# MachinaIO/mxx

Hardware: AMD Instinct MI355X
Metric: dcrt_ring_ops_per_s (higher is better)
Workload: dtype u32

## Files before the change

### mxx_amd/csrc/common.h

```cpp
#pragma once

#include <hip/hip_runtime.h>

#include <atomic>
#include <cstddef>
#include <cstdint>
#include <cstdio>
#include <exception>
#include <map>
#include <unordered_map>
#include <mutex>
#include <string>
#include <vector>

#include "../../include/gpupoly.h"

constexpr size_t GPUPOLY_MAX_LIMBS = 64;

struct LimbConst {
    uint64_t q;
    uint64_t mu;
    uint64_t mu64;
    uint64_t n_inv;
    uint64_t n_inv_sh;
    uint64_t mu32;
    uint64_t inv_last_w;
    uint64_t inv_last_w_sh;
    uint32_t kbits;
    uint32_t lazy_terms;
};

struct EnvSwitches {
    int ntt_path = 0;
    int ntt14 = 0;
    bool decompose_fused = true;
    char matmul_path = 0;
    int matmul_tile = 0;
    bool gsamp_simple = false;
    bool gsamp_no_uni = false;
    bool p1_simple = false;
    int sampler_per_lane = 0;
    int sampler_fill_every = 0;
    bool ntt64_int = false;
    int ntt_phase = 0;
    bool serde_general = false;
    bool rng_compat = false;
    bool pack24 = true;
    int skinny24 = 0;
    int skinny24_shape = 0;
    size_t mul_decompose_many_budget = 0;
    size_t mul_decompose_pairs_budget = 0;
    size_t gadget_scalar_budget = 0;
    size_t ggh15_lookup_budget = 0;
    char mul_sum_path = 0;
    size_t crt_recompose_chunk_bytes = size_t(256) << 20;
    void load();
};

struct GpuContext {
    EnvSwitches env;
    int device = 0;
    std::vector<int> gpu_ids;
    uint32_t logN = 0;
    int N = 0;
    int level = 0;
    uint32_t dnum = 0;
    int limb_count = 0;
    bool wide = false;
    int word_bytes = 4;
    uint32_t crt_bits = 0;
    std::vector<uint64_t> moduli;
    hipStream_t stream = nullptr;
    LimbConst *d_limbs = nullptr;
    LimbConst *d_limbs_r = nullptr;
    void *d_tw_fwd = nullptr;
    void *d_tw_fwd_sh = nullptr;
    void *d_tw_inv = nullptr;
    void *d_tw_inv_sh = nullptr;
    void *d_tw2_fwd = nullptr;
    void *d_tw2_inv = nullptr;
    bool lazy_ok = false;
    bool tight_ok = false;
    void *d_tw2s_inv = nullptr;
    bool signed_ok = false;
    void *d_twf_fwd = nullptr, *d_twf_inv = nullptr;
    void *d_flimbs = nullptr;
    bool f64_ok = false;
    uint64_t *d_garner = nullptr;
    std::vector<uint64_t> garner_inv;
    std::vector<LimbConst> limbs;
    hipEvent_t timer_start = nullptr, timer_stop = nullptr;
    std::vector<hipEvent_t> marks;
    std::mutex mutex;
    bool pool_ok = false;
    std::mutex alloc_mutex;
    std::multimap<size_t, void *> free_blocks;
    std::unordered_map<void *, size_t> live_blocks;
    size_t cached_bytes = 0, cache_limit = 0;
    std::atomic<const char *> last_kernel{""};
    bool pack24_ok = false;
    std::mutex layout_mutex;
    std::map<uint32_t, void *> gadget_weights;
    std::map<std::vector<uint64_t>, void *> gadget_const_tables;
};

struct LayoutTag {
    std::atomic<int> v{GPU_MATRIX_LAYOUT_WORDS};
    LayoutTag() = default;
    LayoutTag(const LayoutTag &o) : v(o.v.load(std::memory_order_acquire)) {}
    LayoutTag &operator=(const LayoutTag &o) {
        v.store(o.v.load(std::memory_order_acquire), std::memory_order_release);
        return *this;
    }
};

struct GpuMatrix {
    GpuContext *ctx = nullptr;
    int level = 0;
    size_t rows = 0, cols = 0;
    int format = GPU_POLY_FORMAT_EVAL;
    void *storage = nullptr;
    size_t bytes = 0;
    LayoutTag layout;
    bool borrowed = false;
    GpuMatrix *parent = nullptr;
    int views = 0;
};

struct GpuEventSet {
    std::vector<hipEvent_t> events;
    int device = 0;
    void *staging = nullptr;
    GpuContext *ctx = nullptr;
    void *dev_staging = nullptr;
};

struct GpuP1CovarianceCache {
    GpuContext *ctx = nullptr;
    int level = 0;
    size_t d = 0, m = 0, n = 0;
    double sigma = 0, s = 0, dgg_stddev = 0;
    double *sqrt_var = nullptr;
    double *update_coeff = nullptr;
    void *karney_div = nullptr;
};

struct P1KeyEntry {
    const double *sqrt_var;
    const double *update_coeff;
    const void *karney_div;
};

static inline dim3 item_grid(size_t items, unsigned threads) {
    const size_t blocks = (items + threads - 1) / threads;
    const size_t max_x = (static_cast<size_t>(1) << 31) / threads;
    if (blocks <= max_x) return dim3(static_cast<unsigned>(blocks ? blocks : 1));
    const size_t y = (blocks + max_x - 1) / max_x;
    return dim3(static_cast<unsigned>((blocks + y - 1) / y), static_cast<unsigned>(y));
}
#if defined(__HIPCC__)
__device__ __forceinline__ size_t item_index() {
    return (static_cast<size_t>(blockIdx.y) * gridDim.x + blockIdx.x) * blockDim.x + threadIdx.x;
}
#endif

extern std::atomic<uint64_t> g_kernel_launches;
extern std::atomic<int> g_trace_on;
void trace_launch_begin(const char *name, hipStream_t stream, dim3 grid, dim3 block);
void trace_launch_end(hipStream_t stream);
void trace_set_bytes(double bytes);
#define MXX_TRACE_BYTES(b)                                                                        \
    do {                                                                                          \
        if (g_trace_on.load(std::memory_order_relaxed)) trace_set_bytes(static_cast<double>(b)); \
    } while (0)
#define MXX_LAUNCH(kern, grid, block, lds, strm, ...)                          \
    do {                                                                       \
        g_kernel_launches.fetch_add(1, std::memory_order_relaxed);             \
        const bool mxx_tr_ = g_trace_on.load(std::memory_order_relaxed) != 0;  \
        if (mxx_tr_) trace_launch_begin(#kern, strm, grid, block);             \
        hipLaunchKernelGGL(kern, grid, block, lds, strm, __VA_ARGS__);         \
        if (mxx_tr_) trace_launch_end(strm);                                   \
    } while (0)
#define MXX_TRACED_COPY(name, strm, bytes, stmt)                               \
    do {                                                                       \
        const bool mxx_tr_ = g_trace_on.load(std::memory_order_relaxed) != 0;  \
        if (mxx_tr_) {                                                         \
            trace_set_bytes(static_cast<double>(bytes));                       \
            trace_launch_begin(name, strm, dim3(0), dim3(0));                  \
        }                                                                      \
        stmt;                                                                  \
        if (mxx_tr_) trace_launch_end(strm);                                   \
    } while (0)

int set_error(const char *msg);
int set_error(const std::string &msg);
int set_error(hipError_t err, const char *what);

#define HIP_TRY(expr)                                          \
    do {                                                       \
        hipError_t _e = (expr);                                \
        if (_e != hipSuccess) return set_error(_e, #expr);     \
    } while (0)

template <auto... KERNELS>
static int lds_opt_in(const GpuContext *ctx, size_t lds) {
    static std::atomic<uint64_t> configured{0};
    const uint64_t bit = 1ull << (ctx->device & 63);
    if (lds <= 64 * 1024 || (configured.load() & bit)) return 0;
    for (const void *f : {reinterpret_cast<const void *>(KERNELS)...})
        HIP_TRY(hipFuncSetAttribute(f, hipFuncAttributeMaxDynamicSharedMemorySize, static_cast<int>(lds)));
    configured.fetch_or(bit);
    return 0;
}

extern int (*g_roctx_push)(const char *);
extern int (*g_roctx_pop)();
void roctx_init_once();
struct RoctxScope {
    bool on;
    explicit RoctxScope(const char *name) {
        roctx_init_once();
        on = g_roctx_push != nullptr;
        if (on) g_roctx_push(name);
    }
    ~RoctxScope() {
        if (on) g_roctx_pop();
    }
};

#define ABI_GUARD_BEGIN try { RoctxScope roctx_scope_(__func__);
#define ABI_GUARD_END                                                         \
    }                                                                         \
    catch (const std::exception &e) { return set_error(e.what()); }           \
    catch (...) { return set_error("unknown exception in libgpupoly"); }

inline size_t matrix_polys(const GpuMatrix *m) { return m->rows * m->cols; }
inline size_t matrix_limbs(const GpuMatrix *m) { return static_cast<size_t>(m->level) + 1; }
inline size_t matrix_words(const GpuMatrix *m) { return matrix_polys(m) * matrix_limbs(m) * static_cast<size_t>(m->ctx->N); }

void *words_ptr(const GpuMatrix *m);
const void *packed24_ptr(const GpuMatrix *m, bool *packed);
inline size_t packed24_bytes(const GpuMatrix *m) { return m->bytes / 4 * 3; }
inline bool storage_overlaps(const GpuMatrix *x, const GpuMatrix *y) {
    if (x == y) return true;
    if (!x->storage || !y->storage || x->bytes == 0 || y->bytes == 0) return false;
    const size_t xb = x->layout.v.load(std::memory_order_acquire) == GPU_MATRIX_LAYOUT_PACKED24 ? packed24_bytes(x) : x->bytes;
    const size_t yb = y->layout.v.load(std::memory_order_acquire) == GPU_MATRIX_LAYOUT_PACKED24 ? packed24_bytes(y) : y->bytes;
    const char *xs = static_cast<const char *>(x->storage), *ys = static_cast<const char *>(y->storage);
    return xs < ys + yb && ys < xs + xb;
}
inline bool same_block(const GpuMatrix *x, const GpuMatrix *y) {
    return x == y || (x->storage == y->storage && x->bytes == y->bytes);
}
inline bool partial_overlap(const GpuMatrix *out, const GpuMatrix *operand) {
    return storage_overlaps(out, operand) && !same_block(out, operand);
}
inline bool row_block_overlaps(const GpuMatrix *m, size_t row, size_t rows, const GpuMatrix *y) {
    if (m->layout.v.load(std::memory_order_acquire) == GPU_MATRIX_LAYOUT_PACKED24) return rows && m->cols && storage_overlaps(m, y);
    if (!m->storage) return false;
    const size_t poly_bytes = matrix_limbs(m) * static_cast<size_t>(m->ctx->N) * m->ctx->word_bytes;
    GpuMatrix block;
    block.storage = static_cast<char *>(m->storage) + row * m->cols * poly_bytes;
    block.bytes = rows * m->cols * poly_bytes;
    return storage_overlaps(&block, y);
}
bool pack24_eligible(const GpuMatrix *m);
int pack24_store(GpuMatrix *m, bool ntt);

int sample_impl(GpuMatrix *out, int dist, double sigma, GpuRngSeed seed, size_t full_ncol, size_t col_offset, bool keep_coeff,
                size_t row_offset = 0, uint32_t tower_first = 0, uint32_t tower_count = 0);

struct RngBlockWindow {
    size_t cols, full_ncol, col_offset;
};
int sample_blocks_impl(const char *entry, bool hashed, GpuMatrix *out, int dist_type, const GpuRngSeed *seeds, const GpuHashTags *tags,
                       size_t nblk, int layout, const size_t *seg_cols, const RngBlockWindow *win, const double *sigma = nullptr);
int sample_decomposed_blocks_impl(const char *entry, bool hashed, GpuMatrix *out, int dist_type, const GpuRngSeed *seeds,
                                  const GpuHashTags *tags, size_t nblk, uint32_t base_bits, int small, size_t src_rows, size_t full_ncol,
                                  size_t col_offset);

int hash_tags_check(const char *entry, const GpuHashTags *tags, size_t ntags, size_t *table_bytes);
size_t hash_tags_staged_words(const GpuHashTags *tags, size_t ntags, size_t table_bytes);
void hash_tags_stage(const GpuHashTags *tags, size_t ntags, size_t table_bytes, uint64_t *staging);
int launch_hash_seeds(GpuContext *ctx, GpuRngSeed *d_seeds, const GpuHashTags *tags, size_t ntags, const uint64_t *d_staged);

int ctx_activate(const GpuContext *ctx);
bool ctx_is_registered(const GpuContext *ctx);
int ctx_alloc(GpuContext *ctx, size_t bytes, void **out);
void ctx_free(GpuContext *ctx, void *ptr);
struct CtxBlock {
    GpuContext *ctx;
    void *ptr = nullptr;
    explicit CtxBlock(GpuContext *c) : ctx(c) {}
    CtxBlock(const CtxBlock &) = delete;
    CtxBlock &operator=(const CtxBlock &) = delete;
    ~CtxBlock() {
        if (ptr) ctx_free(ctx, ptr);
    }
    int alloc(size_t bytes) { return ctx_alloc(ctx, bytes, &ptr); }
    void *release() {
        void *p = ptr;
        ptr = nullptr;
        return p;
    }
};
int matrix_check_same_shape(const GpuMatrix *a, const GpuMatrix *b, const char *who);
int coeff_domain_source(const GpuMatrix *mat, CtxBlock &scratch, const void **src);

int launch_ntt(GpuContext *ctx, void *data, size_t vectors, int limbs_per_poly, bool inverse);
int launch_ntt_lds_u32(GpuContext *ctx, uint32_t *data, size_t vectors, uint32_t L, bool inverse);
int launch_ntt_digits_u32(GpuContext *ctx, uint32_t *out, const uint32_t *coeff, size_t out_vectors, uint32_t L,
                          uint32_t src_cols, uint32_t towers, uint32_t dpt, uint32_t base_bits, size_t k, uint32_t td0 = 0);
int launch_ntt_lds_u64(GpuContext *ctx, uint64_t *data, size_t vectors, uint32_t L, bool inverse);
int launch_ntt_digits_u64(GpuContext *ctx, uint64_t *out, const uint64_t *coeff, size_t out_vectors, uint32_t L,
                          uint32_t src_cols, uint32_t towers, uint32_t dpt, uint32_t base_bits, size_t k, uint32_t td0 = 0);
int launch_intt_oop_u32(GpuContext *ctx, uint32_t *out, const uint32_t *in, size_t vectors, uint32_t L);
int launch_ntt_add_u32(GpuContext *ctx, uint32_t *out, const uint32_t *src, const uint32_t *add, size_t vectors, uint32_t L);
int launch_mul_intt_u32(GpuContext *ctx, uint32_t *out, const uint32_t *in, const uint32_t *w, size_t vectors, uint32_t L);
int launch_matmul(GpuMatrix *out, const GpuMatrix *lhs, const GpuMatrix *rhs);
int launch_ntt_fwd_pack24_u32(GpuContext *ctx, uint32_t *out, const uint32_t *in, size_t vectors, uint32_t L);
int launch_matmul_skinny24(GpuMatrix *out, const GpuMatrix *lhs, const GpuMatrix *rhs, bool small_grid);
int skinny24_parse_shape(const char *s);
int launch_matmul_dma_u32(GpuMatrix *out, const GpuMatrix *lhs, const GpuMatrix *rhs);
int launch_matmul_dma32_u32(GpuMatrix *out, const GpuMatrix *lhs, const GpuMatrix *rhs);
int launch_matmul_mfma_u32(GpuMatrix *out, const GpuMatrix *lhs, const GpuMatrix *rhs);
int launch_copy_block(GpuMatrix *out, const GpuMatrix *src, size_t dst_row, size_t dst_col, size_t src_row,
                      size_t src_col, size_t rows, size_t cols, bool add);
int sample_p1_keyed_segments(const GpuP1CovarianceCache *cache, const P1KeyEntry *d_keys, const GpuMatrix *tp2,
                             const GpuRngSeed *seeds, const size_t *seg_cols, size_t nseg, GpuMatrix *out);
int launch_scatter_i64(GpuMatrix *out, const int64_t *vals);
int finish_staged_i64(GpuMatrix *out, CtxBlock &stage, hipError_t launch_err, const char *what, bool transform = true);
```

### mxx_amd/csrc/matmul_skinny24.hip

```cpp
#include "common.h"
#include "matmul_tile.h"
#include "modarith.h"

#include <map>
#include <string>

namespace skinny24 {

typedef uint32_t u32x3 __attribute__((ext_vector_type(3)));
typedef uint32_t u32x4 __attribute__((ext_vector_type(4)));

__device__ __forceinline__ __amdgpu_buffer_rsrc_t row_rsrc(const char *base, uint32_t bytes) {
    return __builtin_amdgcn_make_buffer_rsrc(const_cast<char *>(base), 0, static_cast<int>(bytes), 0x00020000);
}
constexpr int kAuxNT = 2;

__device__ __forceinline__ void unpack4(uint32_t w0, uint32_t w1, uint32_t w2, uint32_t *o) {
    o[0] = w0 & 0xffffffu;
    o[1] = __builtin_amdgcn_alignbit(w1, w0, 24) & 0xffffffu;
    o[2] = __builtin_amdgcn_alignbit(w2, w1, 16) & 0xffffffu;
    o[3] = w2 >> 8;
}

template <int TC, int G, int WPE, int MAP>
__global__ void __launch_bounds__(256, WPE)
    kernel(uint32_t *__restrict__ C, const uint32_t *__restrict__ A, const uint32_t *__restrict__ B, const LimbConst *__restrict__ limbs,
           uint32_t inner, uint32_t cols, uint32_t L, uint32_t N) {
    static_assert((TC == 8 || TC == 4) && TC % G == 0 && (MAP == 12 || MAP == 16), "skinny24 shape");
    const uint32_t limb = blockIdx.z, c0 = blockIdx.y * TC;
    const uint32_t i = (blockIdx.x * blockDim.x + threadIdx.x) * 4;
    if (i >= N) return;
    const LimbConst lc = limbs[limb];
    const uint32_t q = static_cast<uint32_t>(lc.q);

    uint32_t bcol[TC];
#pragma unroll
    for (int c = 0; c < TC; ++c) bcol[c] = ((min(c0 + c, cols - 1)) * L + limb) * N * 3;
    const uint32_t bstep = cols * L * N * 3;
    const char *bk = reinterpret_cast<const char *>(B);
    const char *arow = reinterpret_cast<const char *>(A) + static_cast<size_t>(limb) * N * 4;
    const size_t astep = static_cast<size_t>(L) * N * 4;
    const uint32_t a_off = i * 4;
    const uint32_t lane = threadIdx.x & 63u;
    const uint32_t b_off = MAP == 12 ? i * 3 : (lane < 48 ? (i - lane * 4) * 3 + lane * 16 : bstep);
    __shared__ u32x4 stage[MAP == 16 ? 4 : 1][MAP == 16 ? G : 1][64];
    const uint32_t wave = threadIdx.x >> 6;

    uint64_t acc[TC][4];
#pragma unroll
    for (int c = 0; c < TC; ++c)
#pragma unroll
        for (int s = 0; s < 4; ++s) acc[c][s] = 0;
    const uint32_t lazy = lc.lazy_terms;
    uint32_t pending = 0;
    for (uint32_t k = 0; k < inner; ++k) {
        const u32x4 av = __builtin_amdgcn_raw_buffer_load_b128(row_rsrc(arow, N * 4), a_off, 0, 0);
        arow += astep;
#pragma unroll
        for (int g0 = 0; g0 < TC; g0 += G) {
            uint32_t raw[G][3];
            if constexpr (MAP == 12) {
#pragma unroll
                for (int g = 0; g < G; ++g) {
                    const u32x3 t = __builtin_amdgcn_raw_buffer_load_b96(row_rsrc(bk, bstep), b_off, bcol[g0 + g], kAuxNT);
                    raw[g][0] = t[0];
                    raw[g][1] = t[1];
                    raw[g][2] = t[2];
                }
            } else {
                __builtin_amdgcn_wave_barrier();
                u32x4 t[G];
#pragma unroll
                for (int g = 0; g < G; ++g) t[g] = __builtin_amdgcn_raw_buffer_load_b128(row_rsrc(bk, bstep), b_off, bcol[g0 + g], kAuxNT);
#pragma unroll
                for (int g = 0; g < G; ++g) stage[wave][g][lane] = t[g];
                __builtin_amdgcn_wave_barrier();
#pragma unroll
                for (int g = 0; g < G; ++g) {
                    const uint32_t *p = reinterpret_cast<const uint32_t *>(&stage[wave][g][0]) + lane * 3;
                    raw[g][0] = p[0];
                    raw[g][1] = p[1];
                    raw[g][2] = p[2];
                }
            }
#pragma unroll
            for (int g = 0; g < G; ++g) {
                uint32_t bv[4];
                unpack4(raw[g][0], raw[g][1], raw[g][2], bv);
#pragma unroll
                for (int s = 0; s < 4; ++s) acc[g0 + g][s] += static_cast<uint64_t>(av[s]) * static_cast<uint64_t>(bv[s]);
            }
        }
        bk += bstep;
        if (++pending == lazy) {
            pending = 0;
#pragma unroll
            for (int c = 0; c < TC; ++c)
#pragma unroll
                for (int s = 0; s < 4; ++s) acc[c][s] = reduce_u64_sum(acc[c][s], q, lc.mu64);
        }
    }
#pragma unroll
    for (int c = 0; c < TC; ++c) {
        if (c0 + c >= cols) continue;
        u32x4 o;
#pragma unroll
        for (int s = 0; s < 4; ++s) o[s] = reduce_u64_sum(acc[c][s], q, lc.mu64);
        *reinterpret_cast<u32x4 *>(C + (static_cast<size_t>(c0 + c) * L + limb) * N + i) = o;
    }
}

#define MXX_SKINNY24_SHAPES(X)                                          \
    X(8, 1, 5, 12) X(8, 2, 5, 12) X(8, 4, 5, 12) X(8, 8, 5, 12) X(8, 8, 4, 12)  \
    X(8, 1, 5, 16) X(8, 2, 5, 16) X(8, 4, 5, 16)                        \
    X(4, 1, 8, 12) X(4, 2, 8, 12) X(4, 4, 8, 12) X(4, 1, 8, 16) X(4, 2, 8, 16) X(4, 4, 8, 16)

constexpr int shape_key(int tc, int g, int wpe, int map) { return ((tc * 16 + g) * 16 + wpe) * 32 + map; }

}

int skinny24_parse_shape(const char *s) {
    int v[4] = {0, 0, 0, 0};
    for (int f = 0; f < 4; ++f) {
        if (*s < '0' || *s > '9') return 0;
        while (*s >= '0' && *s <= '9' && v[f] < 100) v[f] = v[f] * 10 + (*s++ - '0');
        if (f < 3 && *s++ != ',') return 0;
    }
    if (*s || v[0] > 15 || v[1] > 15 || v[2] > 15 || v[3] > 31) return 0;
    return skinny24::shape_key(v[0], v[1], v[2], v[3]);
}

static constexpr int kSkinny24Default = skinny24::shape_key(8, 2, 5, 12);

int launch_matmul_skinny24(GpuMatrix *out, const GpuMatrix *lhs, const GpuMatrix *rhs, bool small_grid) {
    using namespace skinny24;
    GpuContext *ctx = out->ctx;
    const EnvSwitches &env = ctx->env;
    if (env.skinny24 == 1 || ctx->wide || lhs->ctx != ctx || rhs->ctx != ctx) return -1;
    const uint32_t inner = static_cast<uint32_t>(lhs->cols), cols = static_cast<uint32_t>(rhs->cols);
    const uint32_t L = static_cast<uint32_t>(matrix_limbs(out)), N = static_cast<uint32_t>(ctx->N);
    if (lhs->rows != 1 || cols < 8 || N < 4) return -1;
    if (static_cast<uint64_t>(cols) * L * N * 3 >= 0xfffffff0ull) return -1;
    if (rhs->layout.v.load(std::memory_order_acquire) != GPU_MATRIX_LAYOUT_PACKED24) return -1;
    const bool force = env.skinny24 == 2;
    int key = force && env.skinny24_shape ? env.skinny24_shape : kSkinny24Default;
    const int tc = key / (16 * 16 * 32);
    const TileGrid g = tc == 4 ? tile_grid<1, 4, 4>(ctx, 1, cols, L, rhs->bytes) : tile_grid<1, 8, 4>(ctx, 1, cols, L, rhs->bytes);
    if (!force && (!g.streamed || small_grid)) return -1;
    if (!tile_grid_fits(1, cols, 1, tc == 4 ? 4 : 8)) return set_error("gpu_matrix_mul: matrix too large");
    const bool fell_back = key % 32 == 16 && N % 256 != 0;
    if (fell_back) key = key - 16 + 12;
    uint32_t *c = static_cast<uint32_t *>(words_ptr(out));
    if (lhs->layout.v.load(std::memory_order_acquire) == GPU_MATRIX_LAYOUT_PACKED24) (void)words_ptr(lhs);
    std::lock_guard<std::mutex> lk(ctx->layout_mutex);
    bool pa = false, pb = false;
    const uint32_t *a = static_cast<const uint32_t *>(packed24_ptr(lhs, &pa)), *b = static_cast<const uint32_t *>(packed24_ptr(rhs, &pb));
    if (pa || !pb) return -1;
    const char *label;
    {
        static std::mutex label_mutex;
        static std::map<int, std::string> labels;
        std::lock_guard<std::mutex> ll(label_mutex);
        std::string &s = labels[key * 2 + (fell_back ? 1 : 0)];
        if (s.empty())
            s = "skinny24::kernel<TC=" + std::to_string(tc) + ",G=" + std::to_string(key / (16 * 32) % 16) + ",WPE=" + std::to_string(key / 32 % 16) +
                ",MAP=" + std::to_string(key % 32) + (fell_back ? " (16 asked: partial wave)" : "") +
                ",nt,packed24 B> (the tile of matmul_kernel<u32,1," + std::to_string(tc) + ",4,nt,packed24 B>, one row x TC columns x 4 slots per lane, " +
                "B streamed once with non-temporal loads, 3-byte residues, " +
                (key % 32 == 16 ? "16-byte requests through a wave-private LDS slice" : "12 bytes per lane") + ")";
        label = s.c_str();
    }
    switch (key) {
#define MXX_SKINNY24_CASE(TC_, G_, WPE_, MAP_)                                                                                               \
    case shape_key(TC_, G_, WPE_, MAP_):                                                                                                     \
        MXX_LAUNCH((kernel<TC_, G_, WPE_, MAP_>), g.grid, dim3(g.threads), 0, ctx->stream, c, a, b, ctx->d_limbs, inner, cols, L, N); \
        break;
        MXX_SKINNY24_SHAPES(MXX_SKINNY24_CASE)
#undef MXX_SKINNY24_CASE
        default: return set_error("gpu_matrix_mul: MXX_HIP_SKINNY24 names a shape that is not instantiated");
    }
    ctx->last_kernel = label;
    HIP_TRY(hipGetLastError());
    return 0;
}
```

### mxx_amd/csrc/runtime.hip

```cpp
#include "common.h"

#include <algorithm>
#include <cstdlib>
#include <iterator>
#include <map>
#include <cstring>
#include <dlfcn.h>

typedef unsigned __int128 u128h;

static thread_local std::string g_last_error;

int set_error(const char *msg) {
    g_last_error = msg ? msg : "unknown error";
    return 1;
}
int set_error(const std::string &msg) {
    g_last_error = msg;
    return 1;
}
int set_error(hipError_t err, const char *what) {
    g_last_error = std::string(what ? what : "hip call") + ": " + hipGetErrorString(err);
    (void)hipGetLastError();
    return 1;
}

extern "C" const char *gpu_last_error(void) { return g_last_error.c_str(); }
extern "C" int gpu_set_last_error(const char *msg) { return set_error(msg); }
std::atomic<uint64_t> g_kernel_launches{0};
extern "C" uint64_t gpupoly_launch_count(void) { return g_kernel_launches.load(std::memory_order_relaxed); }
extern "C" const char *gpupoly_version(void) { return "gpupoly-mi355x 0.1 (gfx950)"; }

std::atomic<int> g_trace_on{0};
namespace {
struct TraceEntry {
    const char *name;
    hipEvent_t e0, e1;
    unsigned long long blocks;
    unsigned threads;
    double bytes;
    int device;
    bool closed;
};
std::mutex g_trace_mutex;
std::vector<TraceEntry> g_trace;
std::map<int, std::vector<hipEvent_t>> g_trace_pool;
std::string g_trace_report;
thread_local double t_trace_bytes = 0;
thread_local long t_trace_open = -1;
hipEvent_t trace_event(int device) {
    std::vector<hipEvent_t> &pool = g_trace_pool[device];
    if (!pool.empty()) {
        hipEvent_t e = pool.back();
        pool.pop_back();
        return e;
    }
    hipEvent_t e = nullptr;
    if (hipEventCreate(&e) != hipSuccess) {
        (void)hipGetLastError();
        return nullptr;
    }
    return e;
}
void trace_event_return(int device, hipEvent_t e) {
    if (e) g_trace_pool[device].push_back(e);
}
}

void trace_set_bytes(double bytes) { t_trace_bytes = bytes; }

void trace_launch_begin(const char *name, hipStream_t stream, dim3 grid, dim3 block) {
    std::lock_guard<std::mutex> lk(g_trace_mutex);
    int device = 0;
    (void)hipGetDevice(&device);
    TraceEntry en{name, trace_event(device), trace_event(device), 1ull * grid.x * grid.y * grid.z, block.x * block.y * block.z,
                  t_trace_bytes, device, false};
    t_trace_bytes = 0;
    t_trace_open = -1;
    if (!en.e0 || !en.e1 || hipEventRecord(en.e0, stream) != hipSuccess) {
        (void)hipGetLastError();
        trace_event_return(device, en.e0);
        trace_event_return(device, en.e1);
        return;
    }
    g_trace.push_back(en);
    t_trace_open = static_cast<long>(g_trace.size()) - 1;
}

void trace_launch_end(hipStream_t stream) {
    std::lock_guard<std::mutex> lk(g_trace_mutex);
    if (t_trace_open < 0 || static_cast<size_t>(t_trace_open) >= g_trace.size()) return;
    TraceEntry &en = g_trace[static_cast<size_t>(t_trace_open)];
    en.closed = hipEventRecord(en.e1, stream) == hipSuccess;
    if (!en.closed) (void)hipGetLastError();
    t_trace_open = -1;
}

__global__ void gpupoly_marker_kernel(uint32_t id, uint32_t *sink) {
    if (sink && id == 0xffffffffu) *sink = id;
}
extern "C" int gpupoly_marker_launch(GpuContext *ctx, uint32_t id) {
    ABI_GUARD_BEGIN
    if (!ctx) return set_error("gpupoly_marker_launch: null ctx");
    if (ctx_activate(ctx)) return 1;
    hipLaunchKernelGGL(gpupoly_marker_kernel, dim3(1), dim3(1), 0, ctx->stream, id & 0x7fffffffu, static_cast<uint32_t *>(nullptr));
    HIP_TRY(hipGetLastError());
    return 0;
    ABI_GUARD_END
}

extern "C" int gpupoly_trace_begin(void) {
    ABI_GUARD_BEGIN
    std::lock_guard<std::mutex> lk(g_trace_mutex);
    for (const TraceEntry &en : g_trace) {
        trace_event_return(en.device, en.e0);
        trace_event_return(en.device, en.e1);
    }
    g_trace.clear();
    g_trace_on.store(1, std::memory_order_relaxed);
    return 0;
    ABI_GUARD_END
}

extern "C" const char *gpupoly_trace_end(void) {
    try {
        g_trace_on.store(0, std::memory_order_relaxed);
        std::lock_guard<std::mutex> lk(g_trace_mutex);
        g_trace_report.clear();
        int prev = 0;
        (void)hipGetDevice(&prev);
        char line[512];
        for (const TraceEntry &en : g_trace) {
            if (!en.closed) continue;
            (void)hipSetDevice(en.device);
            float ms = 0;
            hipError_t e = hipEventSynchronize(en.e1);
            if (e == hipSuccess) e = hipEventElapsedTime(&ms, en.e0, en.e1);
            if (e != hipSuccess) {
                (void)hipSetDevice(prev);
                set_error(e, "gpupoly_trace_end: hipEventElapsedTime");
                return nullptr;
            }
            std::snprintf(line, sizeof line, "%s\t%llu\t%u\t%.0f\t%.6f\n", en.name, en.blocks, en.threads, en.bytes, ms);
            g_trace_report += line;
        }
        for (const TraceEntry &en : g_trace) {
            trace_event_return(en.device, en.e0);
            trace_event_return(en.device, en.e1);
        }
        g_trace.clear();
        (void)hipSetDevice(prev);
        return g_trace_report.c_str();
    } catch (...) {
        set_error("gpupoly_trace_end: exception");
        return nullptr;
    }
}

int (*g_roctx_push)(const char *) = nullptr;
int (*g_roctx_pop)() = nullptr;
void roctx_init_once() {
    static std::once_flag once;
    std::call_once(once, [] {
        const char *sw = std::getenv("MXX_HIP_ROCTX");
        const bool profiled = std::getenv("ROCP_TOOL_LIBRARIES") != nullptr || std::getenv("ROCPROFILER_REGISTER_FORCE_LOAD") != nullptr;
        if (sw ? sw[0] == '0' : !profiled) return;
        for (const char *name : {"librocprofiler-sdk-roctx.so.1", "librocprofiler-sdk-roctx.so", "libroctx64.so.4", "libroctx64.so"}) {
            void *h = dlopen(name, RTLD_NOW | RTLD_GLOBAL);
            if (!h) continue;
            auto push = reinterpret_cast<int (*)(const char *)>(dlsym(h, "roctxRangePushA"));
            auto pop = reinterpret_cast<int (*)()>(dlsym(h, "roctxRangePop"));
            if (push && pop) {
                g_roctx_pop = pop;
                g_roctx_push = push;
                return;
            }
        }
    });
}

static inline uint64_t h_mulmod(uint64_t a, uint64_t b, uint64_t q) { return (uint64_t)(((u128h)a * b) % q); }
static uint64_t h_powmod(uint64_t b, uint64_t e, uint64_t q) {
    uint64_t r = 1 % q;
    b %= q;
    while (e) {
        if (e & 1) r = h_mulmod(r, b, q);
        b = h_mulmod(b, b, q);
        e >>= 1;
    }
    return r;
}
static uint64_t h_invmod_prime(uint64_t a, uint64_t q) { return h_powmod(a % q, q - 2, q); }

static bool h_is_prime(uint64_t n) {
    static const uint64_t bases[] = {2, 3, 5, 7, 11, 13, 17, 19, 23, 29, 31, 37};
    if (n < 2) return false;
    for (uint64_t b : bases)
        if (n % b == 0) return n == b;
    uint64_t d = n - 1;
    int s = 0;
    while (!(d & 1)) { d >>= 1; ++s; }
    for (uint64_t b : bases) {
        uint64_t x = h_powmod(b, d, n);
        if (x == 1 || x == n - 1) continue;
        bool comp = true;
        for (int r = 1; r < s; ++r) {
            x = h_mulmod(x, x, n);
            if (x == n - 1) { comp = false; break; }
        }
        if (comp) return false;
    }
    return true;
}

static uint64_t h_min_primitive_root(uint64_t q, uint64_t order) {
    uint64_t qm1 = q - 1;
    int v = __builtin_ctzll(qm1);
    int want = __builtin_ctzll(order);
    uint64_t odd = qm1 >> v;
    uint64_t maximal = 0;
    for (uint64_t x = 2; x < q; ++x) {
        uint64_t r = h_powmod(x, odd, q);
        if (h_powmod(r, 1ull << (v - 1), q) != 1) { maximal = r; break; }
    }
    uint64_t root = h_powmod(maximal, 1ull << (v - want), q);
    uint64_t sq = h_mulmod(root, root, q);
    uint64_t cur = root, best = root;
    for (uint64_t i = 1; i < order / 2; ++i) {
        cur = h_mulmod(cur, sq, q);
        if (cur < best) best = cur;
    }
    return best;
}

static inline uint32_t h_bitrev(uint32_t x, uint32_t bits) {
    uint32_t r = 0;
    for (uint32_t i = 0; i < bits; ++i) { r = (r << 1) | (x & 1); x >>= 1; }
    return r;
}
static inline uint32_t h_bits(uint64_t v) { return v ? 64 - (uint32_t)__builtin_clzll(v) : 0; }

void EnvSwitches::load() {
    *this = EnvSwitches();
    if (const char *e = std::getenv("MXX_HIP_NTT_PATH")) {
        if (e[0] == 'l') ntt_path = 1;
        else if (e[0] == 'g' && e[1] == 'e') ntt_path = 2;
        else if (e[0] == 'g' && e[1] == 'l') ntt_path = 3;
    }
    if (const char *e = std::getenv("MXX_HIP_NTT14")) ntt14 = e[0] == 'w' ? 1 : (e[0] == 'u' ? 2 : 0);
    if (const char *e = std::getenv("MXX_HIP_DECOMPOSE_FUSED")) decompose_fused = e[0] != '0';
    if (const char *e = std::getenv("MXX_HIP_MATMUL_PATH")) matmul_path = e[0];
    if (const char *e = std::getenv("MXX_HIP_MATMUL_TILE")) {
        if (e[0] && e[1] && e[2]) matmul_tile = ((e[0] - '0') * 100 + (e[1] - '0') * 10 + (e[2] - '0')) * 2 + (e[3] == 'p');
    }
    if (const char *e = std::getenv("MXX_HIP_GSAMP")) {
        gsamp_simple = e[0] == 's';
        gsamp_no_uni = e[0] == 'n';
    }
    if (const char *e = std::getenv("MXX_HIP_P1")) p1_simple = e[0] == 's';
    if (const char *e = std::getenv("MXX_HIP_NTT64")) ntt64_int = e[0] == 'i';
    if (const char *e = std::getenv("MXX_HIP_RNG_COMPAT")) rng_compat = e[0] == 'r';
    if (const char *e = std::getenv("MXX_HIP_SERDE")) serde_general = e[0] == 'g';
    if (const char *e = std::getenv("MXX_HIP_PACK24")) pack24 = !(std::strcmp(e, "0") == 0 || std::strcmp(e, "off") == 0);
    if (const char *e = std::getenv("MXX_HIP_SKINNY24")) {
        if (std::strcmp(e, "0") == 0) skinny24 = 1;
        else if (std::strncmp(e, "force", 5) == 0 && (e[5] == 0 || e[5] == ':')) {
            skinny24 = 2;
            if (e[5] == ':') skinny24_shape = skinny24_parse_shape(e + 6) ? skinny24_parse_shape(e + 6) : -1;
        }
    }
    if (const char *e = std::getenv("MXX_HIP_MUL_DECOMPOSE_MANY_BUDGET")) mul_decompose_many_budget = static_cast<size_t>(std::strtoull(e, nullptr, 10));
    if (const char *e = std::getenv("MXX_HIP_MUL_DECOMPOSE_PAIRS_BUDGET")) mul_decompose_pairs_budget = static_cast<size_t>(std::strtoull(e, nullptr, 10));
    if (const char *e = std::getenv("MXX_HIP_GADGET_SCALAR_BUDGET")) gadget_scalar_budget = static_cast<size_t>(std::strtoull(e, nullptr, 10));
    if (const char *e = std::getenv("MXX_HIP_GGH15_LOOKUP_BUDGET")) ggh15_lookup_budget = static_cast<size_t>(std::strtoull(e, nullptr, 10));
    if (const char *e = std::getenv("MXX_HIP_CRT_RECOMPOSE_CHUNK_BYTES")) {
        const size_t v = static_cast<size_t>(std::strtoull(e, nullptr, 10));
        if (v >= 1) crt_recompose_chunk_bytes = v;
    }
    if (const char *e = std::getenv("MXX_HIP_MUL_SUM_PATH")) mul_sum_path = (e[0] == 't' || e[0] == 's') ? e[0] : 0;
    if (const char *e = std::getenv("MXX_HIP_SAMPLER_PER_LANE")) {
        const int v = std::atoi(e);
        if (v >= 1 && v <= 4096) sampler_per_lane = v;
    }
    if (const char *e = std::getenv("MXX_HIP_NTT_PHASE")) {
        const int v = std::atoi(e);
        if (v >= 0 && v <= 127) ntt_phase = v;
    }
    if (const char *e = std::getenv("MXX_HIP_SAMPLER_FILL_EVERY")) {
        const int v = std::atoi(e);
        if (v >= 1 && v <= 8) sampler_fill_every = v;
    }
}

static std::mutex g_registry_mutex;
static std::vector<GpuContext *> g_contexts;
bool ctx_is_registered(const GpuContext *ctx) {
    std::lock_guard<std::mutex> lk(g_registry_mutex);
    return std::find(g_contexts.begin(), g_contexts.end(), ctx) != g_contexts.end();
}

extern "C" int gpupoly_reload_env(void) {
    std::lock_guard<std::mutex> lk(g_registry_mutex);
    for (GpuContext *c : g_contexts) c->env.load();
    return 0;
}

int ctx_activate(const GpuContext *ctx) {
    HIP_TRY(hipSetDevice(ctx->device));
    return 0;
}

static size_t round_block(size_t bytes) {
    const size_t gran = bytes >= (size_t(1) << 20) ? (size_t(1) << 20) : 4096;
    return (bytes + gran - 1) / gran * gran;
}

static void cache_trim(GpuContext *ctx, size_t limit) {
    while (ctx->cached_bytes > limit && !ctx->free_blocks.empty()) {
        auto it = std::prev(ctx->free_blocks.end());
        (void)hipFree(it->second);
        ctx->cached_bytes -= it->first;
        ctx->free_blocks.erase(it);
    }
}

int ctx_alloc(GpuContext *ctx, size_t bytes, void **out) {
    *out = nullptr;
    if (bytes == 0) return 0;
    const size_t want = round_block(bytes);
    std::lock_guard<std::mutex> lk(ctx->alloc_mutex);
    auto it = ctx->free_blocks.lower_bound(want);
    if (it != ctx->free_blocks.end() && it->first <= want + want / 4) {
        *out = it->second;
        ctx->live_blocks[*out] = it->first;
        ctx->cached_bytes -= it->first;
        ctx->free_blocks.erase(it);
        return 0;
    }
    hipError_t e = hipMalloc(out, want);
    if (e != hipSuccess) {
        (void)hipGetLastError();
        cache_trim(ctx, 0);
        e = hipMalloc(out, want);
    }
    if (e != hipSuccess) {
        (void)hipGetLastError();
        {
            std::lock_guard<std::mutex> reg(g_registry_mutex);
            for (GpuContext *other : g_contexts) {
                if (other == ctx || other->device != ctx->device) continue;
                if (!other->alloc_mutex.try_lock()) continue;
                cache_trim(other, 0);
                other->alloc_mutex.unlock();
            }
        }
        e = hipMalloc(out, want);
        if (e != hipSuccess) {
            *out = nullptr;
            return set_error(e, "hipMalloc");
        }
    }
    ctx->live_blocks[*out] = want;
    return 0;
}

void ctx_free(GpuContext *ctx, void *ptr) {
    if (!ptr) return;
    std::lock_guard<std::mutex> lk(ctx->alloc_mutex);
    auto it = ctx->live_blocks.find(ptr);
    if (it == ctx->live_blocks.end()) {
        (void)hipFree(ptr);
        return;
    }
    const size_t size = it->second;
    ctx->live_blocks.erase(it);
    if (!ctx->pool_ok) {
        (void)hipFree(ptr);
        return;
    }
    ctx->free_blocks.emplace(size, ptr);
    ctx->cached_bytes += size;
    cache_trim(ctx, ctx->cache_limit);
}

template <typename W>
static int upload_tables(GpuContext *ctx, const std::vector<std::vector<uint64_t>> &fwd,
                         const std::vector<std::vector<uint64_t>> &inv) {
    const size_t N = ctx->N, L = ctx->limb_count;
    const unsigned shift = sizeof(W) * 8;
    std::vector<W> h_f(L * N), h_fs(L * N), h_i(L * N), h_is(L * N);
    for (size_t l = 0; l < L; ++l) {
        uint64_t q = ctx->moduli[l];
        for (size_t j = 0; j < N; ++j) {
            h_f[l * N + j] = (W)fwd[l][j];
            h_fs[l * N + j] = (W)(((u128h)fwd[l][j] << shift) / q);
            h_i[l * N + j] = (W)inv[l][j];
            h_is[l * N + j] = (W)(((u128h)inv[l][j] << shift) / q);
        }
    }
    size_t bytes = L * N * sizeof(W);
    HIP_TRY(hipMalloc(&ctx->d_tw_fwd, bytes));
    HIP_TRY(hipMalloc(&ctx->d_tw_fwd_sh, bytes));
    HIP_TRY(hipMalloc(&ctx->d_tw_inv, bytes));
    HIP_TRY(hipMalloc(&ctx->d_tw_inv_sh, bytes));
    HIP_TRY(hipMemcpy(ctx->d_tw_fwd, h_f.data(), bytes, hipMemcpyHostToDevice));
    HIP_TRY(hipMemcpy(ctx->d_tw_fwd_sh, h_fs.data(), bytes, hipMemcpyHostToDevice));
    HIP_TRY(hipMemcpy(ctx->d_tw_inv, h_i.data(), bytes, hipMemcpyHostToDevice));
    HIP_TRY(hipMemcpy(ctx->d_tw_inv_sh, h_is.data(), bytes, hipMemcpyHostToDevice));
    std::vector<W> h_pf(2 * L * N), h_pi(2 * L * N);
    for (size_t i = 0; i < L * N; ++i) {
        h_pf[2 * i] = static_cast<W>(0) - h_f[i];
        h_pf[2 * i + 1] = h_fs[i];
        h_pi[2 * i] = h_i[i];
        h_pi[2 * i + 1] = h_is[i];
    }
    HIP_TRY(hipMalloc(&ctx->d_tw2_fwd, 2 * bytes));
    HIP_TRY(hipMalloc(&ctx->d_tw2_inv, 2 * bytes));
    HIP_TRY(hipMemcpy(ctx->d_tw2_fwd, h_pf.data(), 2 * bytes, hipMemcpyHostToDevice));
    HIP_TRY(hipMemcpy(ctx->d_tw2_inv, h_pi.data(), 2 * bytes, hipMemcpyHostToDevice));
    if (sizeof(W) == 8 && ctx->crt_bits <= 51 && N >= 2) {
        struct HostTwF { double w, wi; };
        struct HostF64Limb { double q, qinv; HostTwF n_inv, last_w; };
        std::vector<HostTwF> tf(L * N), ti(L * N);
        std::vector<HostF64Limb> fl(L);
        for (size_t l = 0; l < L; ++l) {
            const double qd = static_cast<double>(ctx->moduli[l]);
            for (size_t j = 0; j < N; ++j) {
                tf[l * N + j] = {static_cast<double>(fwd[l][j]), static_cast<double>(fwd[l][j]) / qd};
                ti[l * N + j] = {static_cast<double>(inv[l][j]), static_cast<double>(inv[l][j]) / qd};
            }
            const LimbConst &lc = ctx->limbs[l];
            fl[l] = {qd, 1.0 / qd, {static_cast<double>(lc.n_inv), static_cast<double>(lc.n_inv) / qd},
                     {static_cast<double>(lc.inv_last_w), static_cast<double>(lc.inv_last_w) / qd}};
        }
        HIP_TRY(hipMalloc(&ctx->d_twf_fwd, sizeof(HostTwF) * L * N));
        HIP_TRY(hipMalloc(&ctx->d_twf_inv, sizeof(HostTwF) * L * N));
        HIP_TRY(hipMalloc(&ctx->d_flimbs, sizeof(HostF64Limb) * L));
        HIP_TRY(hipMemcpy(ctx->d_twf_fwd, tf.data(), sizeof(HostTwF) * L * N, hipMemcpyHostToDevice));
        HIP_TRY(hipMemcpy(ctx->d_twf_inv, ti.data(), sizeof(HostTwF) * L * N, hipMemcpyHostToDevice));
        HIP_TRY(hipMemcpy(ctx->d_flimbs, fl.data(), sizeof(HostF64Limb) * L, hipMemcpyHostToDevice));
        ctx->f64_ok = true;
    }
    if (ctx->signed_ok && sizeof(W) == 4) {
        auto signed_pair = [](uint64_t w, uint64_t q, W *dst) {
            const int64_t c = w > q / 2 ? static_cast<int64_t>(w) - static_cast<int64_t>(q) : static_cast<int64_t>(w);
            __int128 num = static_cast<__int128>(c) << 32;
            __int128 fl = num / static_cast<__int128>(q);
            if (num % static_cast<__int128>(q) < 0) fl -= 1;
            dst[0] = static_cast<W>(static_cast<uint32_t>(static_cast<int32_t>(c)));
            dst[1] = static_cast<W>(static_cast<uint32_t>(static_cast<int32_t>(fl)));
        };
        for (size_t l = 0; l < L; ++l)
            for (size_t j = 0; j < N; ++j) signed_pair(inv[l][j], ctx->moduli[l], &h_pi[2 * (l * N + j)]);
        HIP_TRY(hipMalloc(&ctx->d_tw2s_inv, 2 * bytes));
        HIP_TRY(hipMemcpy(ctx->d_tw2s_inv, h_pi.data(), 2 * bytes, hipMemcpyHostToDevice));
    }
    return 0;
}

static void context_release(GpuContext *ctx) {
    if (!ctx) return;
    {
        std::lock_guard<std::mutex> reg(g_registry_mutex);
        g_contexts.erase(std::remove(g_contexts.begin(), g_contexts.end(), ctx), g_contexts.end());
    }
    (void)hipSetDevice(ctx->device);
    if (ctx->stream) (void)hipStreamSynchronize(ctx->stream);
    for (auto &kv : ctx->free_blocks) (void)hipFree(kv.second);
    for (auto &kv : ctx->live_blocks) (void)hipFree(kv.first);
    if (ctx->d_limbs) (void)hipFree(ctx->d_limbs);
    if (ctx->d_limbs_r) (void)hipFree(ctx->d_limbs_r);
    if (ctx->d_twf_fwd) (void)hipFree(ctx->d_twf_fwd);
    if (ctx->d_twf_inv) (void)hipFree(ctx->d_twf_inv);
    if (ctx->d_flimbs) (void)hipFree(ctx->d_flimbs);
    if (ctx->d_tw_fwd) (void)hipFree(ctx->d_tw_fwd);
    if (ctx->d_tw_fwd_sh) (void)hipFree(ctx->d_tw_fwd_sh);
    if (ctx->d_tw_inv) (void)hipFree(ctx->d_tw_inv);
    if (ctx->d_tw_inv_sh) (void)hipFree(ctx->d_tw_inv_sh);
    if (ctx->d_garner) (void)hipFree(ctx->d_garner);
    if (ctx->d_tw2_fwd) (void)hipFree(ctx->d_tw2_fwd);
    if (ctx->d_tw2_inv) (void)hipFree(ctx->d_tw2_inv);
    if (ctx->d_tw2s_inv) (void)hipFree(ctx->d_tw2s_inv);
    for (auto &kv : ctx->gadget_weights) (void)hipFree(kv.second);
    for (auto &kv : ctx->gadget_const_tables) (void)hipFree(kv.second);
    if (ctx->timer_start) (void)hipEventDestroy(ctx->timer_start);
    if (ctx->timer_stop) (void)hipEventDestroy(ctx->timer_stop);
    for (hipEvent_t ev : ctx->marks)
        if (ev) (void)hipEventDestroy(ev);
    if (ctx->stream) (void)hipStreamDestroy(ctx->stream);
    delete ctx;
}

extern "C" int gpu_context_create(uint32_t logN, uint32_t L, uint32_t dnum, const uint64_t *moduli,
                                  size_t moduli_len, const int *gpu_ids, size_t gpu_ids_len, GpuContext **out_ctx) {
    ABI_GUARD_BEGIN
    if (!out_ctx) return set_error("gpu_context_create: null out_ctx");
    *out_ctx = nullptr;
    if (!moduli || moduli_len == 0) return set_error("gpu_context_create: empty moduli");
    if (moduli_len != static_cast<size_t>(L) + 1) return set_error("gpu_context_create: moduli_len must equal L+1");
    if (moduli_len > GPUPOLY_MAX_LIMBS) return set_error("gpu_context_create: too many limbs");
    if (!gpu_ids || gpu_ids_len == 0) return set_error("gpu_context_create: empty gpu_ids");
    if (logN < 1 || logN > 17) return set_error("gpu_context_create: logN out of range [1,17]");
    int dev_count = 0;
    HIP_TRY(hipGetDeviceCount(&dev_count));
    for (size_t i = 0; i < gpu_ids_len; ++i) {
        if (gpu_ids[i] < 0 || gpu_ids[i] >= dev_count) return set_error("gpu_context_create: invalid gpu id");
        for (size_t j = 0; j < i; ++j)
            if (gpu_ids[j] == gpu_ids[i]) return set_error("gpu_context_create: duplicate gpu id");
    }
    const uint64_t N = 1ull << logN;
    bool wide = false;
    for (size_t i = 0; i < moduli_len; ++i) {
        uint64_t q = moduli[i];
        if (q < 3 || (q - 1) % (2 * N) != 0) return set_error("gpu_context_create: modulus must be = 1 (mod 2N)");
        if (!h_is_prime(q)) return set_error("gpu_context_create: modulus is not prime");
        if (q >> 62) return set_error("gpu_context_create: modulus must be < 2^62");
        if (q >> 31) wide = true;
        for (size_t j = 0; j < i; ++j)
            if (moduli[j] == q) return set_error("gpu_context_create: duplicate modulus");
    }

    GpuContext *ctx = new GpuContext();
    ctx->device = gpu_ids[0];
    ctx->gpu_ids.assign(gpu_ids, gpu_ids + gpu_ids_len);
    ctx->logN = logN;
    ctx->N = static_cast<int>(N);
    ctx->level = static_cast<int>(L);
    ctx->dnum = dnum;
    ctx->limb_count = static_cast<int>(moduli_len);
    ctx->wide = wide;
    ctx->word_bytes = wide ? 8 : 4;
    ctx->moduli.assign(moduli, moduli + moduli_len);

    hipError_t e = hipSetDevice(ctx->device);
    if (e != hipSuccess) { delete ctx; return set_error(e, "hipSetDevice"); }
    e = hipStreamCreateWithFlags(&ctx->stream, hipStreamNonBlocking);
    if (e != hipSuccess) { delete ctx; return set_error(e, "hipStreamCreate"); }

    ctx->env.load();
    {
        ctx->pool_ok = true;
        size_t free_b = 0, total_b = 0;
        ctx->cache_limit = size_t(64) << 30;
        if (hipMemGetInfo(&free_b, &total_b) == hipSuccess && free_b) ctx->cache_limit = free_b / 2;
        else (void)hipGetLastError();
        const char *env = std::getenv("MXX_HIP_MEMPOOL_RELEASE_THRESHOLD_BYTES");
        if (!env) env = std::getenv("MXX_CUDA_MEMPOOL_RELEASE_THRESHOLD_BYTES");
        if (env && *env) ctx->cache_limit = std::strtoull(env, nullptr, 10);
        const char *nopool = std::getenv("MXX_HIP_DISABLE_MEMPOOL");
        if (nopool && *nopool == '1') ctx->pool_ok = false;
    }

    std::vector<std::vector<uint64_t>> fwd(moduli_len), inv(moduli_len);
    ctx->limbs.resize(moduli_len);
    uint32_t crt_bits = 0;
    for (size_t l = 0; l < moduli_len; ++l) {
        uint64_t q = moduli[l];
        uint64_t psi = h_min_primitive_root(q, 2 * N);
        uint64_t ipsi = h_invmod_prime(psi, q);
        fwd[l].resize(N);
        inv[l].resize(N);
        uint64_t p = 1, ip = 1;
        for (uint64_t i = 0; i < N; ++i) {
            uint32_t r = h_bitrev(static_cast<uint32_t>(i), logN);
            fwd[l][r] = p;
            inv[l][r] = ip;
            p = h_mulmod(p, psi, q);
            ip = h_mulmod(ip, ipsi, q);
        }
        LimbConst &lc = ctx->limbs[l];
        lc.q = q;
        lc.kbits = h_bits(q);
// ... 245 lines not shown
```

Before: 7.796 million.

## Split last wave of skinny24 matmul into narrower column tiles

Adds a unit-indexed kernel variant that runs the final (limb, column-tile) pairs of the skinny24 matmul with smaller TS-column tiles. The goal is to reduce the partial last wave (tail) when the workgroup count is not a multiple of resident capacity. An auto heuristic uses the CU count and fixed cost constants to pick TS and how many pairs to split. This costs extra B re-reads for the fine tiles and some index arithmetic per block.

```diff
diff --git a/mxx_amd/csrc/common.h b/mxx_amd/csrc/common.h
--- a/mxx_amd/csrc/common.h
+++ b/mxx_amd/csrc/common.h
@@ -48,6 +48,9 @@
     bool pack24 = true;
     int skinny24 = 0;
     int skinny24_shape = 0;
+    int skinny24_tail = 0;
+    int skinny24_tail_ts = 0;
+    int skinny24_tail_pct = 0;
     size_t mul_decompose_many_budget = 0;
     size_t mul_decompose_pairs_budget = 0;
     size_t gadget_scalar_budget = 0;
@@ -320,6 +323,7 @@
 int launch_matmul(GpuMatrix *out, const GpuMatrix *lhs, const GpuMatrix *rhs);
 int launch_ntt_fwd_pack24_u32(GpuContext *ctx, uint32_t *out, const uint32_t *in, size_t vectors, uint32_t L);
 int launch_matmul_skinny24(GpuMatrix *out, const GpuMatrix *lhs, const GpuMatrix *rhs, bool small_grid);
+bool skinny24_parse_tail(const char *s, int *ts, int *pct);
 int skinny24_parse_shape(const char *s);
 int launch_matmul_dma_u32(GpuMatrix *out, const GpuMatrix *lhs, const GpuMatrix *rhs);
 int launch_matmul_dma32_u32(GpuMatrix *out, const GpuMatrix *lhs, const GpuMatrix *rhs);
diff --git a/mxx_amd/csrc/matmul_skinny24.hip b/mxx_amd/csrc/matmul_skinny24.hip
--- a/mxx_amd/csrc/matmul_skinny24.hip
+++ b/mxx_amd/csrc/matmul_skinny24.hip
@@ -1,7 +1,10 @@
 #include "common.h"
 #include "matmul_tile.h"
 #include "modarith.h"
-
+#include "skinny24_units.h"
+
+#include <array>
+#include <atomic>
 #include <map>
 #include <string>
 
@@ -22,13 +25,12 @@
     o[3] = w2 >> 8;
 }
 
-template <int TC, int G, int WPE, int MAP>
-__global__ void __launch_bounds__(256, WPE)
-    kernel(uint32_t *__restrict__ C, const uint32_t *__restrict__ A, const uint32_t *__restrict__ B, const LimbConst *__restrict__ limbs,
-           uint32_t inner, uint32_t cols, uint32_t L, uint32_t N) {
-    static_assert((TC == 8 || TC == 4) && TC % G == 0 && (MAP == 12 || MAP == 16), "skinny24 shape");
-    const uint32_t limb = blockIdx.z, c0 = blockIdx.y * TC;
-    const uint32_t i = (blockIdx.x * blockDim.x + threadIdx.x) * 4;
+template <int TC, int G, int MAP>
+__device__ __forceinline__ void tile(uint32_t *__restrict__ C, const uint32_t *__restrict__ A, const uint32_t *__restrict__ B,
+                                     const LimbConst *__restrict__ limbs, uint32_t inner, uint32_t cols, uint32_t L, uint32_t N, uint32_t limb,
+                                     uint32_t c0, uint32_t chunk, u32x4 *stage) {
+    static_assert((TC == 8 || TC == 4 || TC == 2 || TC == 1) && TC % G == 0 && (MAP == 12 || MAP == 16), "skinny24 shape");
+    const uint32_t i = (chunk * blockDim.x + threadIdx.x) * 4;
     if (i >= N) return;
     const LimbConst lc = limbs[limb];
     const uint32_t q = static_cast<uint32_t>(lc.q);
@@ -43,7 +45,6 @@
     const uint32_t a_off = i * 4;
     const uint32_t lane = threadIdx.x & 63u;
     const uint32_t b_off = MAP == 12 ? i * 3 : (lane < 48 ? (i - lane * 4) * 3 + lane * 16 : bstep);
-    __shared__ u32x4 stage[MAP == 16 ? 4 : 1][MAP == 16 ? G : 1][64];
     const uint32_t wave = threadIdx.x >> 6;
 
     uint64_t acc[TC][4];
@@ -73,11 +74,11 @@
 #pragma unroll
                 for (int g = 0; g < G; ++g) t[g] = __builtin_amdgcn_raw_buffer_load_b128(row_rsrc(bk, bstep), b_off, bcol[g0 + g], kAuxNT);
 #pragma unroll
-                for (int g = 0; g < G; ++g) stage[wave][g][lane] = t[g];
+                for (int g = 0; g < G; ++g) stage[(wave * G + g) * 64 + lane] = t[g];
                 __builtin_amdgcn_wave_barrier();
 #pragma unroll
                 for (int g = 0; g < G; ++g) {
-                    const uint32_t *p = reinterpret_cast<const uint32_t *>(&stage[wave][g][0]) + lane * 3;
+                    const uint32_t *p = reinterpret_cast<const uint32_t *>(stage + (wave * G + g) * 64) + lane * 3;
                     raw[g][0] = p[0];
                     raw[g][1] = p[1];
                     raw[g][2] = p[2];
@@ -110,12 +111,41 @@
     }
 }
 
+#define MXX_SKINNY24_STAGE(G_, MAP_) __shared__ u32x4 stage[(MAP_ == 16 ? 4 * G_ : 1) * 64]
+
+template <int TC, int G, int WPE, int MAP>
+__global__ void __launch_bounds__(256, WPE)
+    kernel(uint32_t *__restrict__ C, const uint32_t *__restrict__ A, const uint32_t *__restrict__ B, const LimbConst *__restrict__ limbs,
+           uint32_t inner, uint32_t cols, uint32_t L, uint32_t N) {
+    MXX_SKINNY24_STAGE(G, MAP);
+    tile<TC, G, MAP>(C, A, B, limbs, inner, cols, L, N, blockIdx.z, blockIdx.y * TC, blockIdx.x, stage);
+}
+
+template <int TC, int G, int WPE, int MAP, int TS>
+__global__ void __launch_bounds__(256, WPE)
+    kernel_units(uint32_t *__restrict__ C, const uint32_t *__restrict__ A, const uint32_t *__restrict__ B, const LimbConst *__restrict__ limbs,
+                 uint32_t inner, uint32_t cols, uint32_t L, uint32_t N, const Skinny24Units units) {
+    static_assert(TS <= TC && TC % TS == 0, "skinny24 tail");
+    MXX_SKINNY24_STAGE(G, MAP);
+    const Skinny24Unit u = skinny24_unit(units, blockIdx.x);
+    if (!u.fine) tile<TC, G, MAP>(C, A, B, limbs, inner, cols, L, N, u.limb, u.c0, u.chunk, stage);
+    else tile<TS, (G < TS ? G : TS), MAP>(C, A, B, limbs, inner, cols, L, N, u.limb, u.c0, u.chunk, stage);
+}
+
 #define MXX_SKINNY24_SHAPES(X)                                          \
     X(8, 1, 5, 12) X(8, 2, 5, 12) X(8, 4, 5, 12) X(8, 8, 5, 12) X(8, 8, 4, 12)  \
     X(8, 1, 5, 16) X(8, 2, 5, 16) X(8, 4, 5, 16)                        \
     X(4, 1, 8, 12) X(4, 2, 8, 12) X(4, 4, 8, 12) X(4, 1, 8, 16) X(4, 2, 8, 16) X(4, 4, 8, 16)
 
 constexpr int shape_key(int tc, int g, int wpe, int map) { return ((tc * 16 + g) * 16 + wpe) * 32 + map; }
+
+constexpr bool shape_instantiated(int key) {
+#define MXX_SKINNY24_IS(TC_, G_, WPE_, MAP_) \
+    if (key == shape_key(TC_, G_, WPE_, MAP_)) return true;
+    MXX_SKINNY24_SHAPES(MXX_SKINNY24_IS)
+#undef MXX_SKINNY24_IS
+    return false;
+}
 
 }
 
@@ -130,7 +160,29 @@
     return skinny24::shape_key(v[0], v[1], v[2], v[3]);
 }
 
+bool skinny24_parse_tail(const char *s, int *ts, int *pct) {
+    if ((s[0] != '4' && s[0] != '2' && s[0] != '1') || s[1] != ',' || s[2] < '0' || s[2] > '9') return false;
+    int v = 0;
+    const char *d = s + 2;
+    while (*d >= '0' && *d <= '9' && v <= 100) v = v * 10 + (*d++ - '0');
+    if (*d || v > 100) return false;
+    *ts = s[0] - '0';
+    *pct = v;
+    return true;
+}
+
 static constexpr int kSkinny24Default = skinny24::shape_key(8, 2, 5, 12);
+
+static uint32_t device_cu_count(int device) {
+    static std::atomic<int> known[64];
+    const bool slot = device >= 0 && device < 64;
+    int cus = slot ? known[device].load(std::memory_order_relaxed) : 0;
+    if (cus < 1) {
+        if (hipDeviceGetAttribute(&cus, hipDeviceAttributeMultiprocessorCount, device) != hipSuccess || cus < 1) cus = 256;
+        if (slot) known[device].store(cus, std::memory_order_relaxed);
+    }
+    return static_cast<uint32_t>(cus);
+}
 
 int launch_matmul_skinny24(GpuMatrix *out, const GpuMatrix *lhs, const GpuMatrix *rhs, bool small_grid) {
     using namespace skinny24;
@@ -150,35 +202,64 @@
     if (!tile_grid_fits(1, cols, 1, tc == 4 ? 4 : 8)) return set_error("gpu_matrix_mul: matrix too large");
     const bool fell_back = key % 32 == 16 && N % 256 != 0;
     if (fell_back) key = key - 16 + 12;
+    if (!shape_instantiated(key)) return set_error("gpu_matrix_mul: MXX_HIP_SKINNY24 names a shape that is not instantiated");
+    if (env.skinny24_tail < 0) return set_error("gpu_matrix_mul: MXX_HIP_SKINNY24_TAIL names a tail that is not instantiated");
     uint32_t *c = static_cast<uint32_t *>(words_ptr(out));
     if (lhs->layout.v.load(std::memory_order_acquire) == GPU_MATRIX_LAYOUT_PACKED24) (void)words_ptr(lhs);
     std::lock_guard<std::mutex> lk(ctx->layout_mutex);
     bool pa = false, pb = false;
     const uint32_t *a = static_cast<const uint32_t *>(packed24_ptr(lhs, &pa)), *b = static_cast<const uint32_t *>(packed24_ptr(rhs, &pb));
     if (pa || !pb) return -1;
+    const uint32_t threads_per_wg = g.threads, chunks = g.grid.x;
+    const uint64_t pairs = static_cast<uint64_t>(g.col_tiles) * L;
+    uint32_t ts = 0;
+    uint64_t fine_pairs = 0;
+    if (env.skinny24_tail == 2) {
+        ts = static_cast<uint32_t>(env.skinny24_tail_ts);
+        fine_pairs = skinny24_fine_pairs_of_pct(pairs, static_cast<uint32_t>(env.skinny24_tail_pct));
+    } else if (env.skinny24_tail == 0) {
+        const uint64_t resident = static_cast<uint64_t>(key / 32 % 16) * 4 / ((threads_per_wg + 63) / 64) * device_cu_count(ctx->device);
+        fine_pairs = skinny24_auto_tail(pairs * chunks, resident, chunks, static_cast<uint32_t>(tc), &ts);
+    }
+    if (fine_pairs > pairs) fine_pairs = pairs;
+    Skinny24Units units = {};
+    if (fine_pairs) {
+        units = skinny24_units(chunks, cols, L, static_cast<uint32_t>(tc), ts, fine_pairs);
+        if (units.units > 0x7fffffffull) fine_pairs = 0;
+    }
     const char *label;
     {
         static std::mutex label_mutex;
-        static std::map<int, std::string> labels;
+        static std::map<std::array<uint64_t, 3>, std::string> labels;
         std::lock_guard<std::mutex> ll(label_mutex);
-        std::string &s = labels[key * 2 + (fell_back ? 1 : 0)];
+        std::string &s = labels[{static_cast<uint64_t>(key * 2 + (fell_back ? 1 : 0)) * 8 + (fine_pairs ? ts : 0), fine_pairs, pairs}];
         if (s.empty())
             s = "skinny24::kernel<TC=" + std::to_string(tc) + ",G=" + std::to_string(key / (16 * 32) % 16) + ",WPE=" + std::to_string(key / 32 % 16) +
                 ",MAP=" + std::to_string(key % 32) + (fell_back ? " (16 asked: partial wave)" : "") +
+                (fine_pairs ? ",TS=" + std::to_string(ts) + ",fine=" + std::to_string(fine_pairs) + "/" + std::to_string(pairs) + " pairs" : std::string()) +
                 ",nt,packed24 B> (the tile of matmul_kernel<u32,1," + std::to_string(tc) + ",4,nt,packed24 B>, one row x TC columns x 4 slots per lane, " +
                 "B streamed once with non-temporal loads, 3-byte residues, " +
-                (key % 32 == 16 ? "16-byte requests through a wave-private LDS slice" : "12 bytes per lane") + ")";
+                (key % 32 == 16 ? "16-byte requests through a wave-private LDS slice" : "12 bytes per lane") +
+                (fine_pairs ? ", the last pairs of the launch in tiles of TS columns" : "") + ")";
         label = s.c_str();
     }
+#define MXX_SKINNY24_ARGS c, a, b, ctx->d_limbs, inner, cols, L, N
+#define MXX_SKINNY24_UNITS(TC_, G_, WPE_, MAP_, TS_) \
+    MXX_LAUNCH((kernel_units<TC_, G_, WPE_, MAP_, TS_>), dim3(static_cast<uint32_t>(units.units)), dim3(g.threads), 0, ctx->stream, MXX_SKINNY24_ARGS, units)
     switch (key) {
-#define MXX_SKINNY24_CASE(TC_, G_, WPE_, MAP_)                                                                                               \
-    case shape_key(TC_, G_, WPE_, MAP_):                                                                                                     \
-        MXX_LAUNCH((kernel<TC_, G_, WPE_, MAP_>), g.grid, dim3(g.threads), 0, ctx->stream, c, a, b, ctx->d_limbs, inner, cols, L, N); \
+#define MXX_SKINNY24_CASE(TC_, G_, WPE_, MAP_)                                                                       \
+    case shape_key(TC_, G_, WPE_, MAP_):                                                                             \
+        if (!fine_pairs) MXX_LAUNCH((kernel<TC_, G_, WPE_, MAP_>), g.grid, dim3(g.threads), 0, ctx->stream, MXX_SKINNY24_ARGS); \
+        else if (ts == 4) MXX_SKINNY24_UNITS(TC_, G_, WPE_, MAP_, 4);                                                \
+        else if (ts == 2) MXX_SKINNY24_UNITS(TC_, G_, WPE_, MAP_, 2);                                                \
+        else MXX_SKINNY24_UNITS(TC_, G_, WPE_, MAP_, 1);                                                             \
         break;
         MXX_SKINNY24_SHAPES(MXX_SKINNY24_CASE)
 #undef MXX_SKINNY24_CASE
         default: return set_error("gpu_matrix_mul: MXX_HIP_SKINNY24 names a shape that is not instantiated");
     }
+#undef MXX_SKINNY24_UNITS
+#undef MXX_SKINNY24_ARGS
     ctx->last_kernel = label;
     HIP_TRY(hipGetLastError());
     return 0;
diff --git a/mxx_amd/csrc/runtime.hip b/mxx_amd/csrc/runtime.hip
--- a/mxx_amd/csrc/runtime.hip
+++ b/mxx_amd/csrc/runtime.hip
@@ -268,6 +268,11 @@
             skinny24 = 2;
             if (e[5] == ':') skinny24_shape = skinny24_parse_shape(e + 6) ? skinny24_parse_shape(e + 6) : -1;
         }
+    }
+    if (const char *e = std::getenv("MXX_HIP_SKINNY24_TAIL")) {
+        if (std::strcmp(e, "0") == 0) skinny24_tail = 1;
+        else if (std::strcmp(e, "auto") == 0) skinny24_tail = 0;
+        else skinny24_tail = skinny24_parse_tail(e, &skinny24_tail_ts, &skinny24_tail_pct) ? 2 : -1;
     }
     if (const char *e = std::getenv("MXX_HIP_MUL_DECOMPOSE_MANY_BUDGET")) mul_decompose_many_budget = static_cast<size_t>(std::strtoull(e, nullptr, 10));
     if (const char *e = std::getenv("MXX_HIP_MUL_DECOMPOSE_PAIRS_BUDGET")) mul_decompose_pairs_budget = static_cast<size_t>(std::strtoull(e, nullptr, 10));
diff --git a/mxx_amd/csrc/skinny24_units.h b/mxx_amd/csrc/skinny24_units.h
--- /dev/null
+++ b/mxx_amd/csrc/skinny24_units.h
@@ -0,0 +1,80 @@
+#pragma once
+#include <cstdint>
+
+#if defined(__HIPCC__)
+#define MXX_UNITS_HD __host__ __device__ __forceinline__
+#else
+#define MXX_UNITS_HD inline
+#endif
+
+struct Skinny24Units {
+    uint32_t chunks;
+    uint32_t col_tiles;
+    uint32_t tc, ts;
+    uint32_t subs;
+    uint32_t pairs_big;
+    uint32_t u_big;
+    uint32_t sub0;
+    uint64_t units;
+};
+
+struct Skinny24Unit {
+    uint32_t limb, c0, chunk;
+    bool fine;
+};
+
+MXX_UNITS_HD Skinny24Units skinny24_units(uint32_t chunks, uint32_t cols, uint32_t L, uint32_t tc, uint32_t ts, uint64_t fine_pairs) {
+    Skinny24Units p;
+    p.chunks = chunks;
+    p.col_tiles = (cols + tc - 1) / tc;
+    p.tc = tc;
+    p.ts = ts;
+    p.subs = (cols + ts - 1) / ts;
+    const uint64_t pairs = static_cast<uint64_t>(L) * p.col_tiles;
+    if (fine_pairs > pairs) fine_pairs = pairs;
+    p.pairs_big = static_cast<uint32_t>(pairs - fine_pairs);
+    p.u_big = p.pairs_big * chunks;
+    const uint32_t limb0 = p.pairs_big / p.col_tiles, tile0 = p.pairs_big % p.col_tiles;
+    p.sub0 = limb0 * p.subs + tile0 * (tc / ts);
+    p.units = static_cast<uint64_t>(p.pairs_big) * chunks + (static_cast<uint64_t>(L) * p.subs - p.sub0) * chunks;
+    return p;
+}
+
+MXX_UNITS_HD Skinny24Unit skinny24_unit(const Skinny24Units &p, uint32_t u) {
+    Skinny24Unit r;
+    r.fine = u >= p.u_big;
+    if (!r.fine) {
+        const uint32_t pair = u / p.chunks;
+        r.chunk = u - pair * p.chunks;
+        r.limb = pair / p.col_tiles;
+        r.c0 = (pair - r.limb * p.col_tiles) * p.tc;
+    } else {
+        const uint32_t v = u - p.u_big, w = v / p.chunks, s = p.sub0 + w;
+        r.chunk = v - w * p.chunks;
+        r.limb = s / p.subs;
+        r.c0 = (s - r.limb * p.subs) * p.ts;
+    }
+    return r;
+}
+
+constexpr uint32_t kTailSlow[3] = {1370, 1220, 1140};
+MXX_UNITS_HD uint64_t skinny24_auto_tail(uint64_t units, uint64_t resident, uint32_t chunks, uint32_t tc, uint32_t *ts) {
+    *ts = 0;
+    if (resident == 0 || units <= resident) return 0;
+    const uint64_t r = units % resident;
+    if (r == 0) return 0;
+    uint64_t best = 750ull * tc;
+    for (uint32_t i = 0, t = 1; i < 3 && t < tc; ++i, t *= 2) {
+        const uint64_t rounds = (r * (tc / t) + resident - 1) / resident;
+        const uint64_t cost = rounds * t * kTailSlow[i];
+        if (cost < best) {
+            best = cost;
+            *ts = t;
+        }
+    }
+    if (*ts == 0) return 0;
+    const uint64_t rp = (r + chunks - 1) / chunks;
+    return rp + (rp + 7) / 8 + 1;
+}
+
+MXX_UNITS_HD uint64_t skinny24_fine_pairs_of_pct(uint64_t pairs, uint32_t pct) { return (pairs * pct + 50) / 100; }
```

Result: no change. 7.806 million, median of 4 (+0.1%).
